# Yukayo/MobGT

Measured on AMD Instinct MI355X. Metric: check-ins/sec (train step), higher is better.
Workload: dtype bf16

## Files before the change

### __graft_entry__.py

```python
import os
import subprocess
import sys

ROOT = os.path.dirname(os.path.abspath(__file__))
if ROOT not in sys.path:
    sys.path.insert(0, ROOT)


def build() -> None:
    from mobgt_amd import _native
    for library in _native.LIBRARIES:
        library.build()
        library.lib()
    from mobgt_amd import _pairbins
    _pairbins.LIBRARY.build()
    _pairbins.LIBRARY.lib()
    from mobgt_amd import _universe
    _universe.LIBRARY.build()
    _universe.LIBRARY.lib()
    from mobgt_amd import _checkins
    _checkins.LIBRARY.build()
    _checkins.LIBRARY.lib()
    from mobgt_amd import _prefixes
    _prefixes.LIBRARY.build()
    _prefixes.LIBRARY.lib()
    from mobgt_amd import _baseline
    _baseline.LIBRARY.build()
    _baseline.LIBRARY.lib()
    from mobgt_amd import _prior
    _prior.LIBRARY.build()
    _prior.LIBRARY.lib()
    from mobgt_amd import _geoprior
    _geoprior.LIBRARY.build()
    _geoprior.LIBRARY.lib()
    from mobgt_amd import _priorfit
    _priorfit.LIBRARY.build()
    _priorfit.LIBRARY.lib()
    from mobgt_amd import _ctxprior
    _ctxprior.LIBRARY.build()
    _ctxprior.LIBRARY.lib()
    from mobgt_amd import _tokhost
    _tokhost.LIBRARY.build()
    _tokhost.LIBRARY.lib()
    from mobgt_amd import _visitprior
    _visitprior.LIBRARY.build()
    _visitprior.LIBRARY.lib()
    subprocess.check_call(["make", "-s", "-C", os.path.join(ROOT, "oracle")])
    import mobgt_amd


def smoke() -> None:
    import numpy as np
    import torch
    from mobgt_amd import ops, synth
    from mobgt_amd.model_fqandtoyo import EncoderLayer
    from oracle import algos_oracle as ao
    from oracle import model_oracle as mo
    assert torch.cuda.is_available(), "smoke() needs cuda:0"
    dev = "cuda:0"
    G, H, T, C = 3, 8, 37, 192
    torch.manual_seed(0)
    layer = EncoderLayer(C, 256, 0.1, 0.1, H).eval()
    sd = {"L." + k: v.detach().clone().requires_grad_(True) for k, v in layer.state_dict().items()}
    rng = np.random.RandomState(0)
    x = torch.from_numpy(rng.standard_normal((G, T, C)).astype(np.float32))
    gy = torch.from_numpy(rng.standard_normal((G, T, C)).astype(np.float32))
    bias = torch.from_numpy((rng.standard_normal((G, H, T, T)) * 0.5).astype(np.float32))
    bias[1, :, :, 30:] = float("-inf")
    xr, br = x.clone().requires_grad_(True), bias.clone().requires_grad_(True)
    ref = mo.encoder_layer_fq(sd, "L", xr, br, H)
    ref.backward(gy)
    layer = layer.to(dev)
    xd, bd = x.to(dev).requires_grad_(True), bias.to(dev).requires_grad_(True)
    out = layer(xd, bd)
    out.backward(gy.to(dev))
    torch.cuda.synchronize()

    def close(name, got, want, tol):
        got, want = got.detach().float().cpu().numpy(), want.detach().numpy()
# ... 40 lines not shown
```

### mobgt_amd/csrc/sgemm_body.h

```cpp
#pragma once
#include "common.h"
#include "mobgt_hip.h"

namespace mobgt_sgemm {

typedef __attribute__((ext_vector_type(4))) float f32x4;

struct SgemmParams {
    const float* A; int64_t lda;
    const float* B; int64_t ldb;
    const float* bias;
    void* C; int64_t ldc;
    int c_bf16;
    int M, N, K;
    int act;
    float slope;
    uint32_t thr;
    float inv_keep;
    uint64_t seed;
    const uint64_t* seed_dev;
    uint32_t salt;
    const float* amask;
    float mpos, mneg, mzero;
    bf16_t* ct;
// ... 45 lines not shown
        acc = __builtin_amdgcn_mfma_f32_16x16x4f32(a_r[u].w, b_r[u].w, acc, 0, 0, 0);
    }
#pragma unroll
    for (int v = 0; v < 4; ++v) part[wave][(4 * kq + v) * 17 + i] = acc[v];
    __syncthreads();
    if (wave == 0) {
    const uint64_t seed = p.thr ? p.seed + (p.seed_dev ? *p.seed_dev : 0ull) : 0ull;
    const int c = i;
    const float bv = (p.bias && c < p.N) ? p.bias[c] : 0.f;
#pragma unroll
    for (int v = 0; v < 4; ++v) {
        const int r = m0 + 4 * kq + v;
        if (r >= p.M || c >= p.N) continue;
        float o = bv;
#pragma unroll
        for (int w = 0; w < KS; ++w) o += part[w][(4 * kq + v) * 17 + i];
        if (p.act) {
            o = o > 0.f ? o : p.slope * o;
            if (p.thr) {
                const uint32_t rowh = dropout_row_hash(seed, (uint32_t)r ^ p.salt);
                o = dropout_bits16(seed, rowh, (uint32_t)c) >= p.thr ? o * p.inv_keep : 0.f;
            }
        }
        if (p.C) {
            if (p.c_bf16) reinterpret_cast<bf16_t*>(p.C)[(int64_t)r * p.ldc + c] = (bf16_t)o;
            else reinterpret_cast<float*>(p.C)[(int64_t)r * p.ldc + c] = o;
        }
        if (p.ct) p.ct[(int64_t)c * p.ldt + r] = (bf16_t)(p.ct_scale ? o * p.ct_scale[r] : o);
    }
    }
    __syncthreads();
}

}
```

### mobgt_amd/forms.py

```python
import contextlib
import os
from collections import namedtuple

Form = namedtuple("Form", "name env default doc")

_ROWS = (
    Form("safe_forms", "MOBGT_SAFE_FORMS", False, "no launch waits for peer workgroups: one workgroup per row block, the head as "
         "three launches, the GCN layer by layer (what TrainStep.guarded_step switches to before it re-runs a faulted step)"),
    Form("chain", "MOBGT_NO_CHAIN", True, "out-proj -> LN -> FFN -> LN -> the next layer's QKV in one launch (off: separate launches)"),
    Form("chain_big", "MOBGT_NO_CHAIN_BIG", True, "past 4 096 rows: the 64-row forward chain (off: the library's GEMMs)"),
    Form("chain_bwd", None, True, "the same chain backwards, d(out) -> d(attention out)"),
    Form("ln_gemm", None, True, "dropout+residual+LN as the prologue of the GEMM that consumes it (off: the two-launch form)"),
    Form("ln_gemm_bwd", "MOBGT_LN_GEMM_BWD", False, "the LayerNorm-prologue GEMMs in the backward as well"),
    Form("own_gemm", None, True, "the layer's GEMMs on csrc/gemm.hip (off: through torch)"),
    Form("tail", None, True, "a layer's input-gradient GEMM rides in its grouped weight-gradient launch"),
    Form("defer_tail", "MOBGT_NO_DEFER_TAIL", True, "a layer leaves dx and its weight gradients to the chain_bwd launch of the layer "
         "below (off: it finishes its own backward)"),
    Form("wgrad_big", None, True, "past 4 096 rows: the layer's weight gradients as one launch"),
    Form("skinny_all", "MOBGT_SKINNY_ALL", False, "all three classifier products on csrc/skinny.hip (off: dW / db only)"),
    Form("token_fwd_chain", "MOBGT_NO_TOKEN_FWD_CHAIN", True, "the encoder input's forward as one launch (off: four)"),
    Form("token_bwd_chain", "MOBGT_NO_TOKEN_BWD_CHAIN", True, "the encoder input's backward as one launch, csrc/tokbwd.hip (off: three)"),
    Form("l0_token_host", "MOBGT_NO_L0_TOKEN_HOST", True, "the first encoder layer leaves dx and its weight gradients to the encoder "
         "input's one-launch backward (off: it finishes its own backward); no workgroup waits for another, so safe_forms keeps it"),
    Form("l0_token_host_eager", "MOBGT_L0_TOKEN_HOST_EAGER", False, "l0_token_host outside a graph capture as well (off: only a step "
         "that is being captured defers; an eager step is bound by the host, gains nothing and keeps its launch list)"),
    Form("pack_passenger", "MOBGT_NO_PACK_PASSENGER", True, "the layers' weight pack, in the next front launch"),
    Form("front_passengers", "MOBGT_NO_FRONT_PASSENGERS", True, "hop table forward and node-feature indices, in the category GCN's forward"),
    Form("bias_bwd_passenger", "MOBGT_NO_BIAS_BWD_PASSENGER", True, "short batches: the bias tables' backward, in the category GCN's backward"),
    Form("bias_bwd_beside", None, True, "long batches: the bias tables' backward on a side stream (off: where autograd reaches it)"),
    Form("l0_ride", "MOBGT_NO_L0_RIDE", True, "the distance GCN's first product, in the bias assembly's launch"),
    Form("psum_defer", "MOBGT_NO_PSUM_DEFER", True, "split-K partial sums, in the step's one reduction launch into the gradient sinks"),
    Form("small_gcn", "MOBGT_NO_SMALL_GCN", True, "the three-layer category GCN as one launch each way (off: layer by layer)"),
    Form("conv_act", "MOBGT_NO_CONV_ACT", True, "bias + LeakyReLU + dropout in the small GEMM's epilogue (off: launch per product)"),
    Form("dist_gcn_fused", "MOBGT_NO_DIST_GCN_FUSED", True, "the distance GCN on the masked-GEMM launches"),
    Form("sp_gather", None, True, "sparse adjacency, transposed product as a gather (off: the atomic scatter)"),
    Form("stock_front", "MOBGT_NO_STOCK_FRONT", True, "hop table, weight pack and encoder input as one front launch"),
    Form("stock_tail", "MOBGT_NO_STOCK_TAIL", True, "the encoder input's and the wide hop table's backward share one grid at the flush"),
    Form("stock_ln_qkv", "MOBGT_NO_STOCK_LN_QKV", True, "the first layer's norm inside its QKV GEMM"),
    Form("attn_one_pass", "MOBGT_ATTN_TWO_PASS", True, "T > 64, bf16: one-pass backward (off: the two deterministic passes)"),
    Form("ddp_overlap", "MOBGT_DDP_OVERLAP", False, "the backward split into graphs, finished gradient slices all-reduced beside the next"),
    Form("ddp_host_exchange", "MOBGT_DDP_HOST_EXCHANGE", False, "all-reduce issued by the host between backward and optimizer graph"),
    Form("force_comm", "MOBGT_FORCE_COMM", False, "a process group of one rank takes the data-parallel path (tests)"),
)
_BY_NAME = {row.name: row for row in _ROWS}
_OVERRIDES = {}


def _env_set(var):
    v = os.environ.get(var, "")
    if v in ("", "0"):
        return False
    if v == "1":
        return True
    raise ValueError(f"{var}={v!r}: expected unset, '', '0' or '1'")


def on(name):
    row = _BY_NAME[name]
# ... 30 lines not shown
```

### mobgt_amd/modelGNN.py

```python
import math

import torch
import torch.nn as nn
import torch.nn.functional as F
from torch.nn import Parameter

from . import forms
from .step_state import STEP


def mm_tn_splitk(x, g, max_chunks=32, bf16_operands=False, dw=None):
    if (bf16_operands and x.is_cuda and x.dtype == torch.float32 and g.dtype == torch.float32 and x.shape[1] % 2 == 0
            and g.shape[1] % 2 == 0 and x.is_contiguous() and g.is_contiguous()
            and x.data_ptr() % 8 == 0 and g.data_ptr() % 8 == 0):
        from . import ops
        return ops.linear_wgrad(x, g, leaf=True, dw=dw)[0]
    P = x.shape[0]
    s = max((c for c in range(1, max_chunks + 1) if P % c == 0), default=1)
    if s == 1 or P < 2048:
        return x.t() @ g
    return torch.bmm(x.view(s, P // s, -1).transpose(1, 2), g.view(s, P // s, -1)).sum(0)


_OUT_DTYPE = [None]
# ... 447 lines not shown
                  _p(t2), *[_p(x) for x in grads], _p(scratch[n * H1:]), _p(scratch[:n * H1]),
                  _p(counter), n, K0, H1, H2, H3, slope, p_drop, seed, _p(seed_dev), salt,
                  *extra, _stream())
        if job is not None:
            job["done"] = outs
        return (None, None, None, *grads, None, None, None, None, None, None)


class _DistGcnFn(torch.autograd.Function):

    @staticmethod
    def forward(ctx, ax_pad, mask, mask_t, scale, rows, w0, b0, w1, b1, w2, b2, slope, p_drop, seed, seed_dev, salt):
        from . import ops, _lib
        from .ops import _p, _stream
        P, R, NO = ax_pad.shape[0], rows.numel(), w2.shape[1]
        dev = ax_pad.device
        y0t = xt_workspace(dev, P, 16, slot=0)
        y0 = ops.small_gemm(ax_pad, w0, b0, leaky=slope, k_b=w0.shape[0], ct=(y0t, None, False))
        y1t = xt_workspace(dev, P, 64, slot=0)
        t1 = torch.empty(P, 16, dtype=torch.float32, device=dev)
        y1 = torch.empty(P, 64, dtype=torch.float32, device=dev)
        u = torch.empty(R, 64, dtype=torch.float32, device=dev)
        parts = torch.empty(4, R, NO, dtype=torch.float32, device=dev)
        rs_rows = torch.empty(R, dtype=torch.float32, device=dev)
        _lib.call("mobgt_mask_gemm_l1_fwd", _p(mask), mask.shape[1], _p(scale), _p(y0t), y0t.stride(0), _p(t1), _p(w1), _p(b1),
                  float(slope), float(p_drop), int(seed), _p(seed_dev), int(salt) & 0xFFFFFFFF, _p(y1),
                  _p(y1t), y1t.stride(0), None, 0, P, P, _stream())
        _lib.call("mobgt_mask_rows_fwd", _p(mask), mask.shape[1], _p(rows), _p(scale), _p(y1t), y1t.stride(0), _p(w2), _p(b2),
                  _p(u), _p(parts), _p(rs_rows), R, P, NO, _stream())
        ctx.save_for_backward(ax_pad, y0, t1, y1, u, rs_rows, rows, w0, w1, w2, mask_t, scale)
        ctx.mv0, ctx.mv1 = ops.act_mask_values(slope, 0.0), ops.act_mask_values(slope, p_drop)
        ctx.sinks = tuple(ops.grad_sink(t) for t in (w0, b0, w1, b1, w2, b2))
        p0, rest = parts[0], parts[1:]
        ctx.mark_non_differentiable(rest)
        ctx.set_materialize_grads(False)
        return p0, rest

    @staticmethod
    def backward(ctx, g, _g_rest=None):
        from . import ops, _lib
        from .ops import _p, _stream
        ax_pad, y0, t1, y1, u, rs_rows, rows, w0, w1, w2, mask_t, scale = ctx.saved_tensors
        k_w0, k_b0, k_w1, k_b1, k_w2, k_b2 = ctx.sinks
        if g is None:
            return (None,) * 16
        g = g.contiguous()
        dev = g.device
        P, R = ax_pad.shape[0], rows.numel()

        def dst(k, n):
            return k[:] if k is not None else ops.zeros_f32((n,), dev)
        db2 = dst(k_b2, w2.shape[1])
        dW2 = ops.linear_wgrad_masked(u, g, db=db2, db_of_x=True, leaf=True, dw=k_w2[:] if k_w2 is not None else None)
        gut = xt_workspace(dev, R, 64, slot=2)
        ops.small_gemm(g, w2, b_is_nk=True, ct=(gut, rs_rows, True))
        dy1 = torch.empty(P, 64, dtype=torch.float32, device=dev)
        dtt = xt_workspace(dev, P, 16, slot=1)
        _lib.call("mobgt_mask_rows_bwd", _p(mask_t), mask_t.shape[1], _p(rows), _p(gut), gut.stride(0), _p(y1),
                  float(ctx.mv1[0]), float(ctx.mv1[1]), float(ctx.mv1[2]), _p(w1), _p(scale), _p(dy1),
                  _p(dtt), dtt.stride(0), R, P, _stream())
        db1 = dst(k_b1, 64)
        dW1 = ops.linear_wgrad_masked(t1, dy1, x_mask=y1, mask_vals=ctx.mv1, db=db1, db_of_x=True, leaf=True,
                                      dw=k_w1[:] if k_w1 is not None else None)
        dy0 = mask_gemm(MaskAdj(None, mask_t, scale), None, transposed=True, xt=dtt)
        db0 = dst(k_b0, 16)
        dw_dst = None
        extra = (ax_pad.shape[1] - w0.shape[0]) * w0.shape[1]
        if k_w0 is not None and k_w0.is_contiguous() and 0 <= extra <= 16:
            dw_dst = torch.as_strided(k_w0, (ax_pad.shape[1], w0.shape[1]), (w0.shape[1], 1))
        dW0 = ops.linear_wgrad_masked(ax_pad, dy0, x_mask=y0, mask_vals=ctx.mv0, db=db0, db_of_x=True, leaf=True, dw=dw_dst)
        dW0 = dW0[:w0.shape[0]]
        return (None, None, None, None, None, dW0, db0[:], dW1, db1[:], dW2, db2[:], None, None, None, None, None)


def _dist_gcn_ok(gcn, adj_x_pad, rows, mask_adj):
    if not forms.on("dist_gcn_fused") or adj_x_pad is None or rows is None or mask_adj is None or len(gcn.gcn) != 3:
        return False
    g0, g1, g2 = gcn.gcn
    if not (adj_x_pad.is_cuda and adj_x_pad.dtype == torch.float32 and adj_x_pad.is_contiguous() and adj_x_pad.shape[1] % 16 == 0
            and 0 <= adj_x_pad.shape[1] - g0.in_features < 16):
        return False
    if (g0.out_features, g1.in_features, g1.out_features, g2.in_features) != (16, 16, 64, 64) or g2.out_features % 4 or g2.out_features > 192:
        return False
    for g in (g0, g1, g2):
        if g.bias is None or g.weight.dtype != torch.float32 or not g.weight.is_contiguous() or not g.bias.is_contiguous():
            return False
    P = adj_x_pad.shape[0]
    if rows.dtype != torch.int64 or not rows.is_contiguous() or rows.numel() < 1 or mask_adj.scale.numel() != P:
# ... 16 lines not shown
        n_hidden = len(self.gcn) - 1
        adj_x_pad = None
        if adj_x is not None and adj_x.shape[1] != self.gcn[0].in_features:
            adj_x_pad, adj_x = adj_x, adj_x[:, :self.gcn[0].in_features]
        if rows is None and mask_adj is None and x.is_cuda and _small_gcn_ok(self, x, adj, adj_x, adj_t):
            from . import ops
            p_drop = self.dropout if self.training else 0.0
            g0, g1, g2 = self.gcn
            salt = (0x2000 + g2.out_features) & 0xFFFFFFFF
            pre = STEP.gcn_prelaunched.pop(id(self), None)
            seed_dev = ops.dropout_seed(0.0)[1]
            if pre is not None and (pre[0][0], pre[0][2], pre[0][3]) == (float(p_drop), id(seed_dev), salt):
                seed = pre[0][1]
            else:
                seed, seed_dev = ops.dropout_seed(p_drop)
                if pre is not None:
                    if pre[1][2] is not None:
                        torch.cuda.current_stream().wait_event(pre[1][2])
                    pre = None
            with torch.autocast(device_type="cuda", enabled=False):
                return _SmallGcnFn.apply(adj_x, adj, adj_t, g0.weight, g0.bias, g1.weight, g1.bias, g2.weight, g2.bias,
                                         float(self.leaky_relu.negative_slope), float(p_drop), seed, seed_dev, salt,
                                         pre[1] if pre is not None else None)
        ax_in = adj_x_pad if adj_x_pad is not None else adj_x
        if x.is_cuda and not isinstance(adj, CsrAdj) and _dist_gcn_ok(self, ax_in, rows, mask_adj):
            from . import ops
            p_drop = self.dropout if self.training else 0.0
            seed, seed_dev = ops.dropout_seed(p_drop)
            g0, g1, g2 = self.gcn
            with torch.autocast(device_type="cuda", enabled=False):
                p0, rest = _DistGcnFn.apply(ax_in, mask_adj.mask, mask_adj.mask_t, mask_adj.scale, rows, g0.weight, g0.bias,
                                            g1.weight, g1.bias, g2.weight, g2.bias, float(self.leaky_relu.negative_slope),
                                            float(p_drop), seed, seed_dev, 0x2000 + g2.out_features)
            if parts_ok:
                p0._mobgt_parts = tuple(rest.unbind(0))
                return p0
            return ((p0 + rest[0]) + rest[1]) + rest[2]
        if x.is_cuda and all(g.out_features % 4 == 0 and g.bias is not None for g in self.gcn[:-1]):
            from . import ops
            for i in range(n_hidden):
                p_drop = self.dropout if (i == n_hidden - 1 and self.training) else 0.0
                salt = 0x2000 + self.gcn[-1].out_features
                gc = self.gcn[i]
                pre = adj_x if i == 0 else None
                pre_pad = adj_x_pad if i == 0 else None
                if (pre_pad is not None and mask_adj is not None and not isinstance(adj, CsrAdj) and i + 1 < n_hidden
                        and pre_pad.dtype == torch.float32 and pre_pad.is_contiguous() and pre_pad.shape[1] % 16 == 0
                        and 0 <= pre_pad.shape[1] - gc.in_features < 16 and gc.bias is not None and gc.out_features in (16, 32, 48, 64)
                        and gc.weight.is_contiguous() and forms.on("conv_act")
                        and _conv_act_ok(gc.out_features, self.gcn[i + 1].weight, self.gcn[i + 1].bias)):
                    seed, seed_dev = ops.dropout_seed(p_drop)
                    yt = xt_workspace(pre_pad.device, pre_pad.shape[0], gc.out_features, slot=0)
                    with torch.autocast(device_type="cuda", enabled=False):
                        x = _ConvActFn.apply(None, pre_pad, gc.weight, gc.bias, None, float(self.leaky_relu.negative_slope),
                                             float(p_drop), seed, seed_dev, salt, ops.OutRef(yt))
                    x._mobgt_xt = yt
                    continue
                if (pre is None and mask_adj is not None and not isinstance(adj, CsrAdj) and x.dtype == torch.float32
                        and _mask_conv_ok(x, gc.weight) and _conv_act_ok(x.shape[1], gc.weight, gc.bias)):
                    seed, seed_dev = ops.dropout_seed(p_drop)
                    xt = getattr(x, "_mobgt_xt", None)
                    with torch.autocast(device_type="cuda", enabled=False):
                        x = _ConvActFn.apply(None if pre is not None else x, pre, gc.weight, gc.bias, mask_adj,
                                             float(self.leaky_relu.negative_slope), float(p_drop), seed, seed_dev, salt,
                                             ops.OutRef(xt) if xt is not None else None)
                    continue
# ... 29 lines not shown
```

### mobgt_amd/model_fqandtoyo.py

```python
import os
import pickle

import numpy as np
import torch
import torch.nn as nn
import torch.nn.functional as F

from . import forms, ops
from .restriction import Restriction
from .step_state import STEP
from .lr import PolynomialDecayLR
from .model import (FeedForwardNetwork, MultiHeadAttention, hop_table_from, no_grad_row0, fused_layer_forward,
                    refresh_shadows, flush_pending_pack)
from .modelGNN import GCN, prelaunch_small_gcn

node_dim = 2000


def freedman_diaconis_bins(x, return_bins=False):
    iqr = np.subtract(*np.percentile(x, [75, 25]))
    binsize = 2 * iqr * np.power(len(x), -1 / 3)
    bins = np.ceil((np.max(x) - np.min(x)) / binsize)
    if return_bins:
        return int(bins), np.histogram(x, int(bins))[1]
# ... 276 lines not shown
            hop = self.hop_table(batched_data)
        return ops.build_bias(batched_data.attn_bias, batched_data.rel_pos, batched_data.poi_pos, edge_input,
                              self.rel_pos_encoder.weight, self.poi_pos_encoder.weight, hop,
                              self.graph_token_virtual_distance.weight, D, dtype=self.bias_dtype)

    def node_features(self, batched_data, indices=None):
        G, N = batched_data.x.shape[:2]
        idx, real, rows_only = indices if indices is not None else self.gather_indices(batched_data)
        poi_idx, time_idx, cat_idx, pos_idx, gcn_rows, zero_idx, in_deg, out_deg = idx.unbind(0)
        if self.sparse_adj:
            from .modelGNN import CsrAdj
            adj = CsrAdj(self.D_A_rowptr, self.D_A_col, self.D_A_val, self.D_AT_rowptr, self.D_AT_col, self.D_AT_val)
            poidist = self.poi_distance_model(self.X, adj, self.D_AX, rows=gcn_rows.reshape(-1) if rows_only else None)
        else:
            mask_adj = None
            if getattr(self, "D_mask", None) is not None:
                from .modelGNN import MaskAdj
                mask_adj = MaskAdj(self.D_mask, self.D_mask_t, self.D_scale)
            poidist = self.poi_distance_model(self.X, self.D_A, self.D_AX, rows=gcn_rows.reshape(-1) if rows_only else None,
                                              adj_t=self.D_A_T, mask_adj=mask_adj, parts_ok=G * N <= 4096)
        ops.trace_nan("poidist", poidist)
        catemb = self.poi_cat_model(self.C_X, self.C_A, self.C_AX, adj_t=self.C_A_T)
        Wp, Wt, Wc, C = poidist.shape[1], self.time_embed_model_48.weight.shape[1], catemb.shape[1], self.pos_embed.pe.shape[1]
        f4 = self.embed_fuse_model4
        one_launch = G * N <= 4096
        l0 = self.layers[0]
        first_qkv = None
        if (getattr(l0, "fused", False) and getattr(l0, "_packed_fresh", False) and getattr(l0, "act_dtype", None) == torch.bfloat16
                and not torch.is_autocast_enabled("cuda")):
            first_qkv = (l0._packed[0], l0._shadows[1])
        ops.token_fwd_deferral(one_launch and first_qkv is not None and self.act_dtype == torch.bfloat16 and C == 192 and Wp + Wt == 160)
        try:
            return self._node_features_tail(batched_data, G, N, poidist, catemb, real, one_launch, first_qkv, Wp, Wt, Wc, C,
                                            poi_idx, time_idx, cat_idx, pos_idx, zero_idx, in_deg, out_deg)
        finally:
            ops.token_fwd_deferral(False)

    def _node_features_tail(self, batched_data, G, N, poidist, catemb, real, one_launch, first_qkv, Wp, Wt, Wc, C,
                            poi_idx, time_idx, cat_idx, pos_idx, zero_idx, in_deg, out_deg):
        f4 = self.embed_fuse_model4
        if one_launch:
            pt, x4, add = ops.embed_gather_multi(
                [(poidist, poi_idx, 0, 0, False, None)] +
                [(part, poi_idx, 0, 0, 2, None) for part in getattr(poidist, "_mobgt_parts", ())] +
                [(self.time_embed_model_48.weight, time_idx, 0, Wp, False, self.time_embed_model_48.padding_idx),
                 (catemb, cat_idx, 1, Wp + Wt, False, None),
                 (self.fre_embed_model.weight, zero_idx, 2, 0, False, 0), (self.in_degree_encoder.weight, in_deg, 2, 0, True, 0),
                 (self.out_degree_encoder.weight, out_deg, 2, 0, True, 0), (self.pos_embed.pe, pos_idx, 2, 0, True, None)],
                [Wp + Wt, Wp + Wt + Wc, C])
            f2 = ops.linear_splitk(pt, self.embed_fuse_model2.fuse_embed.weight, self.embed_fuse_model2.fuse_embed.bias,
                                   self.act_dtype == torch.bfloat16, slope=self.embed_fuse_model2.leaky_relu.negative_slope,
                                   out=x4[:, :Wp + Wt])
            if f2.data_ptr() == x4.data_ptr():
                x4 = ops.join_cols(x4, f2)
            else:
                x4 = torch.cat((f2, x4[:, Wp + Wt:]), 1)
            nf = ops.linear_splitk(x4, f4.fuse_embed.weight, f4.fuse_embed.bias, getattr(f4, "bf16_wgrad", False),
                                   slope=f4.leaky_relu.negative_slope)
            if f2.data_ptr() == x4.data_ptr() and self.act_dtype == torch.bfloat16 and getattr(f4, "bf16_wgrad", False):
                ops.register_token_chain(nf, x4, Wp + Wt, f4.fuse_embed.weight, f4.leaky_relu.negative_slope,
                                         self.embed_fuse_model2.fuse_embed.weight, self.embed_fuse_model2.leaky_relu.negative_slope)
        else:
            pt = ops.embed_gather_concat([poidist, self.time_embed_model_48.weight], [poi_idx, time_idx],
                                         padding_idx=[None, self.time_embed_model_48.padding_idx])
            f2 = ops.linear_splitk(pt, self.embed_fuse_model2.fuse_embed.weight, self.embed_fuse_model2.fuse_embed.bias,
                                   self.act_dtype == torch.bfloat16, slope=self.embed_fuse_model2.leaky_relu.negative_slope)
            nf = f4(f2, ops.embed_gather_sum([catemb], [cat_idx]))
            add = ops.embed_gather_sum(
                [self.fre_embed_model.weight, self.in_degree_encoder.weight, self.out_degree_encoder.weight, self.pos_embed.pe],
                [zero_idx, in_deg, out_deg, pos_idx], padding_idx=[0, 0, 0, None])
        ops.trace_nan("pt", pt)
        ops.trace_nan("f2", f2)
        ops.trace_nan("fuse4", nf)
        return ops.assemble_tokens(nf.view(G, N, -1), real, add.view(G, N, -1), self.graph_token.weight, self.pos_embed.pe, self.pos_embed.dropout.p,
                                   self.input_dropout.p, self.training,
                                   bf16_copy=self.act_dtype == torch.bfloat16 and getattr(self.layers[0], "fused", False),
                                   pe_row0_via_gather=one_launch, first_qkv=first_qkv)

    def validate_batch(self, batched_data):
        if getattr(batched_data, "_mobgt_validated", None) is self or not batched_data.x.is_cuda:
            return
        if torch.cuda.is_current_stream_capturing():
# ... 187 lines not shown
```

### mobgt_amd/ops.py

```python
import contextlib
import ctypes
import math

import torch

from . import _lib, _tokhost, forms
from ._lib import F32, BF16, I64, I32, I16, U8, check
from .step_state import STEP

_DT = {torch.float32: F32, torch.bfloat16: BF16}
BIAS_LONG_PAIRS, HOP_DMAX, TOPK_MAX = _lib.LIBRARY.constants("BIAS_LONG_PAIRS", "HOP_DMAX", "TOPK_MAX_K")
SKINNY_MAX_G, SKINNY_MAX_K, SKINNY_MFMA_MAX_K, SKINNY_MFMA_K_STEP = _lib.LIBRARY.constants(
    "SKINNY_MAX_G", "SKINNY_MAX_K", "SKINNY_MFMA_MAX_K", "SKINNY_MFMA_K_STEP")
_IT = {torch.int64: I64, torch.int32: I32, torch.int16: I16, torch.uint8: U8}


def _stream():
    return ctypes.c_void_p(torch.cuda.current_stream().cuda_stream)


def _p(t):
    return ctypes.c_void_p(t.data_ptr()) if t is not None else ctypes.c_void_p(0)


def _require_cuda(*ts):
    for t in ts:
        if t is not None and not t.is_cuda:
            raise RuntimeError("mobgt_amd ops run on the GPU only (there is no CPU fallback); got a CPU tensor")




def _ws_word(ws, off):
    return ws.view(torch.int32)[off // 4:off // 4 + 1]


def _scrub_exchange_area(ws, fault_off):
    ws[fault_off + 4:].zero_()
    torch.cuda.synchronize()
# ... 1151 lines not shown
                  _IT[ctx.idx[0].dtype], _stream())
        return (None, None, *grads, *([None] * n))


def embed_gather_concat(tables, indices, padding_idx=None):
    _require_cuda(*tables, *indices)
    n = len(tables)
    shape = indices[0].shape
    skip = tuple(-1 if (padding_idx is None or padding_idx[t] is None) else int(padding_idx[t]) for t in range(n))
    idx = [i.contiguous().reshape(-1) for i in indices]
    tabs = [t.float().contiguous() for t in tables]
    out = _GatherConcatFn.apply(skip, n, *tabs, *idx)
    return out.view(*shape, out.shape[1])


_ROW0_PENDING = {}


def token_fwd_deferral(on):
    flush_token_fwd()
    STEP.token_fwd_on = bool(on) and forms.on("token_fwd_chain") and not _NAN_TRACE["on"]


def flush_token_fwd():
    for k in ("gather", "f2", "f4"):
        rec = STEP.token_fwd.pop(k, None)
        if rec is not None:
            rec["launch"]()


class _GatherMultiFn(torch.autograd.Function):

    @staticmethod
    def forward(ctx, spec, out_widths, n, *args):
        tables, idx = args[:n], args[n:]
        R = idx[0].numel()
        dev = tables[0].device
        outs = [torch.empty(R, w, dtype=torch.float32, device=dev) for w in out_widths]
        ci, i64, vp = ctypes.c_int, ctypes.c_int64, ctypes.c_void_p

        def launch():
            _lib.call("mobgt_embed_gather_multi",
                n, _ptr_array(tables), None, _ptr_array(idx), (i64 * n)(*[sp[3] for sp in spec]),
                (ci * n)(*[t.shape[1] for t in tables]), (ci * n)(*[sp[1] for sp in spec]), (ci * n)(*[int(sp[2]) for sp in spec]),
                (vp * n)(*[outs[sp[0]].data_ptr() for sp in spec]), (i64 * n)(*[outs[sp[0]].stride(0) for sp in spec]), R,
                _IT[idx[0].dtype], 0, None, 0, _stream())
        if STEP.token_fwd_on and "gather" not in STEP.token_fwd and len(outs) == 3 and all(i_.dtype == idx[0].dtype for i_ in idx):
            STEP.token_fwd["gather"] = dict(launch=launch, tables=tables, idx=idx, spec=spec, outs=outs, R=R)
        else:
            launch()
        ctx.idx, ctx.spec, ctx.n = idx, spec, n
        ctx.ptrs = [t.data_ptr() for t in tables]
        ctx.shapes = [t.shape for t in tables]
        ctx.sinks = [grad_sink(t) for t in tables]
        return tuple(outs)

    @staticmethod
    def backward(ctx, *douts):
        n, spec = ctx.n, ctx.spec
        dev = ctx.idx[0].device
        R = ctx.idx[0].numel()
        gbuf = []
        for g in douts:
            if g is not None and (g.stride(1) != 1 or g.stride(0) % 4 or g.data_ptr() % 16 or g.dtype != torch.float32):
                g = g.float().contiguous()
            gbuf.append(g)
        grads = [(ctx.sinks[t][:] if ctx.sinks[t] is not None else zeros_f32(tuple(sh), dev))
                 if (ctx.needs_input_grad[3 + t] and gbuf[spec[t][0]] is not None) else None for t, sh in enumerate(ctx.shapes)]
        jobs = [t for t in range(n) if grads[t] is not None]
        if jobs:
            m = len(jobs)
            ci, i64, vp = ctypes.c_int, ctypes.c_int64, ctypes.c_void_p
            extra, extra_job = None, 0
            for k, t in enumerate(jobs):
                pend = _ROW0_PENDING.pop(ctx.ptrs[t], None)
                if pend is not None:
                    extra, extra_job = pend, k
            _lib.call("mobgt_embed_gather_multi",
                m, None, (vp * m)(*[grads[t].data_ptr() for t in jobs]), (vp * m)(*[ctx.idx[t].data_ptr() for t in jobs]),
                (i64 * m)(*[spec[t][3] for t in jobs]), (ci * m)(*[ctx.shapes[t][1] for t in jobs]),
                (ci * m)(*[spec[t][1] for t in jobs]), None, (vp * m)(*[gbuf[spec[t][0]].data_ptr() for t in jobs]),
                (i64 * m)(*[gbuf[spec[t][0]].stride(0) for t in jobs]), R, _IT[ctx.idx[0].dtype], 1, _p(extra), extra_job,
                _stream())
        return (None, None, None, *grads, *([None] * n))


def embed_gather_multi(jobs, out_widths):
    n = len(jobs)
    tabs = [j[0].float().contiguous() for j in jobs]
    idx = [j[1].contiguous().reshape(-1) for j in jobs]
    _require_cuda(*tabs, *idx)
    spec = tuple((int(j[2]), int(j[3]), int(j[4]), -1 if j[5] is None else int(j[5])) for j in jobs)
    for k, sp in enumerate(spec):
        assert sp[2] != 2 or (k > 0 and tabs[k].shape[1] == tabs[k - 1].shape[1] and not tabs[k].requires_grad
                              and (k < 4 or any(s_[2] != 2 for s_ in spec[k - 3:k]))), "fold job (at most three per gather)"
    return list(_GatherMultiFn.apply(spec, tuple(out_widths), n, *tabs, *idx))


class _JoinColsFn(torch.autograd.Function):

    @staticmethod
    def forward(ctx, whole, part):
        ctx.w = part.shape[1]
        return whole.detach().view_as(whole)

    @staticmethod
    def backward(ctx, g):
        return g, g[:, :ctx.w]


def join_cols(whole, part):
    return _JoinColsFn.apply(whole, part)


class _GradientTailLossFn(torch.autograd.Function):
    @staticmethod
    def forward(ctx, logits, targets, alpha, target_offset):
        logits = logits.float().contiguous()
        G, V = logits.shape
        dlogits = torch.empty_like(logits)
        loss = torch.empty((), dtype=torch.float32, device=logits.device)
        _lib.call("mobgt_gradient_tail_loss", _p(logits), _p(targets.long().contiguous()), int(target_offset), _p(dlogits),
                  _p(loss), G, V, float(alpha), _stream())
        ctx.save_for_backward(dlogits)
        return loss

    @staticmethod
    def backward(ctx, g):
        (dlogits,) = ctx.saved_tensors
# ... 976 lines not shown
```

### mobgt_amd/step_state.py

```python
import contextlib
from collections import namedtuple

PARKED, CARRIED, SWITCH = "parked", "carried", "switch"
Field = namedtuple("Field", "name scope new doc")
_none = type(None)

FIELDS = (
    Field("zero_arena", SWITCH, _none, "TrainStep._prologue sets the step's ZeroArena; ops.zeros_f32 carves from it"),
    Field("grad_sinks", CARRIED, dict, "TrainStep (ops.set_grad_sinks): parameter address -> (weak parameter, gradient view); ops.grad_sink reads"),
    Field("sink_census", SWITCH, lambda: {"on": False, "cur": {}, "max": {}}, "train.used_parameters' dry run counts ops.grad_sink requests per forward"),
    Field("bias_bwd_job", PARKED, _none, "_BuildBiasFn.forward parks; the category GCN's backward launch, the side stream or its own backward takes"),
    Field("front_on", SWITCH, bool, "the model's forward (ops.front_deferral) around the hop table and the node indices"),
    Field("front_hop", PARKED, _none, "_HopTableFn.forward parks; the category GCN's / stock front's forward launch or ops.flush_front takes"),
    Field("front_ni", PARKED, _none, "ops.node_index parks; the same launches take"),
    Field("token_fwd_on", SWITCH, bool, "model_fqandtoyo.node_features (ops.token_fwd_deferral)"),
    Field("token_fwd", PARKED, dict, "'gather' / 'f2' / 'f4': _GatherMultiFn / _LinearSplitKFn.forward record; _AssembleTokensFn launches them as one"),
    Field("token_fwd_fused_calls", CARRIED, int, "how often mobgt_token_fwd_chain took the three records (a counter for tests)"),
    Field("token_chain", CARRIED, _none, "ops.register_token_chain: the encoder-input chain of the forward that just ran; its backward reads it"),
    Field("token_pending", PARKED, dict, "_AssembleTokensFn.backward parks under a gradient's address (with the first layer's tail, taken from layer_tails, "
          "under 'tail'); FuseEmbeddings-4 / -2's backward re-park / launch"),
    Field("front_sgemm", PARKED, dict, "'job': ops.front_small_gemm parks, the bias assembly's launch takes; 'done': its result until ops.small_gemm asks"),
    Field("wgrad_on", SWITCH, bool, "ops.recording_wgrads around the trainer's backward"),
    Field("wgrad_items", PARKED, list, "leaf weight gradients (ops.linear_wgrad*, fused layers) for ops.flush_deferred_wgrads' grouped launch"),
    Field("wgrad_hop", PARKED, _none, "_HopTableFn.backward parks; rides in the flush's first grouped launch"),
    Field("wgrad_hop_wide", PARKED, _none, "_HopTableFn.backward past 256 edge ids; shares the flush's stock tail launch"),
    Field("wgrad_stock_tok", PARKED, _none, "_StockTokensFn.backward parks; the flush's stock tail launch takes"),
    Field("wgrad_psum", PARKED, list, "ops.defer_partial_sum: split-K partial sums for the flush's one reduction launch"),
    Field("layer_tails", PARKED, dict, "(graph task, device, address of dx1) -> a fused layer's tail; the chain launch of the layer below (first layer: "
          "the encoder input's backward) takes"),
    Field("tail_check_task", PARKED, _none, "graph task whose end-of-backward check (fused_layer._pending_check) is queued"),
    Field("weight_pack", PARKED, list, "model.pack_layer_weights(defer=True) parks; the category GCN's / stock front's forward launch takes"),
    Field("gcn_prelaunched", PARKED, dict, "modelGNN.prelaunch_small_gcn: id(module) -> (key, result); that module's forward adopts it"),
)


class StepState:
    def __init__(self):
        for f in FIELDS:
            setattr(self, f.name, f.new())

    def leftovers(self):
        held = {f.name: getattr(self, f.name) for f in FIELDS if f.scope == PARKED}
        return {k: sorted(map(str, v)) if isinstance(v, dict) else len(v) if isinstance(v, list) else type(v).__name__
                for k, v in held.items() if v is not None and v != [] and v != {}}
# ... 25 lines not shown
```

Baseline: 27230.

## Fuse token-gradient scatters into one burst kernel with distance GCN gu product riding along

Result: faster. 27710 (median of 6 runs) (+1.7%).

```diff
diff --git a/__graft_entry__.py b/__graft_entry__.py
--- a/__graft_entry__.py
+++ b/__graft_entry__.py
@@ -45,6 +45,9 @@
     from mobgt_amd import _visitprior
     _visitprior.LIBRARY.build()
     _visitprior.LIBRARY.lib()
+    from mobgt_amd import _tokscatter
+    _tokscatter.LIBRARY.build()
+    _tokscatter.LIBRARY.lib()
     subprocess.check_call(["make", "-s", "-C", os.path.join(ROOT, "oracle")])
     import mobgt_amd
 
diff --git a/include/mobgt_tokscatter.h b/include/mobgt_tokscatter.h
--- /dev/null
+++ b/include/mobgt_tokscatter.h
@@ -0,0 +1,31 @@
+#ifndef MOBGT_TOKSCATTER_H
+#define MOBGT_TOKSCATTER_H
+#include <stdint.h>
+
+#ifdef __cplusplus
+extern "C" {
+#endif
+
+#define MOBGT_TOKSCATTER_EBADDIM (-1)
+#define MOBGT_TOKSCATTER_EALIGN (-2)
+#define MOBGT_TOKSCATTER_EDTYPE (-3)
+
+#define MOBGT_TOKSCATTER_ABI_VERSION 1
+int mobgt_tokscatter_abi_version(void);
+
+#define MOBGT_TOKSCATTER_I64 0
+#define MOBGT_TOKSCATTER_I32 1
+#define MOBGT_TOKSCATTER_MAX_JOBS 8
+#define MOBGT_TOKSCATTER_MAX_WIDTH 192
+#define MOBGT_TOKSCATTER_RIDE_MAX_K 192
+#define MOBGT_TOKSCATTER_RIDE_MAX_N 64
+
+int mobgt_tokscatter_bwd(int n, float* const* d_tables, const void* const* idx, const int64_t* skip, const int* width,
+                         const int* coff, const float* const* buf, const int64_t* ld, int64_t R, int idx_dtype,
+                         const float* extra_row0, int extra_job, int identity_job, const float* ride_w, int64_t ride_ldw,
+                         const float* ride_scale, void* ride_gut, int64_t ride_ldt, int ride_n, void* stream);
+
+#ifdef __cplusplus
+}
+#endif
+#endif
diff --git a/mobgt_amd/_tokscatter.py b/mobgt_amd/_tokscatter.py
--- /dev/null
+++ b/mobgt_amd/_tokscatter.py
@@ -0,0 +1,16 @@
+from ._native import Library, NativeError
+
+
+class MobgtTokscatterError(NativeError):
+    pass
+
+
+LIBRARY = Library("mobgt_tokscatter.h", "csrc_tokscatter", "libmobgt_tokscatter.so", "MOBGT_TOKSCATTER_", error=MobgtTokscatterError,
+                  missing="the burst scatter runs on the device only (MOBGT_NO_SCATTER_BURST=1 does without).",
+                  errors={"EBADDIM": "size outside the supported limits, null buffer, or an identity job / ride that cannot be",
+                          "EALIGN": "pointer or stride violates the documented alignment", "EDTYPE": "unknown index dtype code"},
+                  extra_inputs=("csrc/sgemm_body.h", "csrc/common.h"))
+lib, launch = LIBRARY.lib, LIBRARY.launch
+SIGNATURES, CONSTANTS, ABI_VERSION = LIBRARY.SIGNATURES, LIBRARY.CONSTANTS, LIBRARY.ABI_VERSION
+MAX_JOBS, MAX_WIDTH, RIDE_MAX_K, RIDE_MAX_N = LIBRARY.constants("MAX_JOBS", "MAX_WIDTH", "RIDE_MAX_K", "RIDE_MAX_N")
+EBADDIM, EALIGN, EDTYPE = LIBRARY.constants("EBADDIM", "EALIGN", "EDTYPE")
diff --git a/mobgt_amd/csrc/sgemm_body.h b/mobgt_amd/csrc/sgemm_body.h
--- a/mobgt_amd/csrc/sgemm_body.h
+++ b/mobgt_amd/csrc/sgemm_body.h
@@ -101,4 +101,49 @@
     __syncthreads();
 }
 
+constexpr int NK_MAXS = 12;
+template <typename TI>
+__device__ __forceinline__ void sgemm_nk_tile_burst(const SgemmParams& p, const int tile, const TI* row_idx, const int64_t skip) {
+    const int lane = threadIdx.x & 63;
+    const int i = lane & 15, kq = lane >> 4;
+    const int tiles_n = (p.N + 15) / 16;
+    const int m0 = (tile / tiles_n) * 16, n0 = (tile % tiles_n) * 16;
+    const int ra = min(m0 + i, p.M - 1);
+    const float* arow = p.A + (int64_t)ra * p.lda + 4 * kq;
+    const float* brow = p.B + (int64_t)min(n0 + i, p.N - 1) * p.ldb + 4 * kq;
+    const int nsteps = p.K / 16;
+    const TI ri_raw = row_idx ? row_idx[ra] : (TI)0;
+    float4 a_r[NK_MAXS], b_r[NK_MAXS];
+#pragma unroll
+    for (int s = 0; s < NK_MAXS; ++s) {
+        const int sc = min(s, nsteps - 1);
+        a_r[s] = *reinterpret_cast<const float4*>(arow + 16 * sc);
+        b_r[s] = *reinterpret_cast<const float4*>(brow + 16 * sc);
+    }
+    float sc_r[4];
+#pragma unroll
+    for (int v = 0; v < 4; ++v) sc_r[v] = p.ct_scale ? p.ct_scale[min(m0 + 4 * kq + v, p.M - 1)] : 1.f;
+    const int64_t ri = (int64_t)ri_raw;
+    const uint32_t keep = (ri < 0 || ri == skip) ? 0u : 0xFFFFFFFFu;
+    f32x4 acc = f32x4{0.f, 0.f, 0.f, 0.f};
+#pragma unroll
+    for (int s = 0; s < NK_MAXS; ++s) {
+        if (s < nsteps) {
+            acc = __builtin_amdgcn_mfma_f32_16x16x4f32(__uint_as_float(__float_as_uint(a_r[s].x) & keep), b_r[s].x, acc, 0, 0, 0);
+            acc = __builtin_amdgcn_mfma_f32_16x16x4f32(__uint_as_float(__float_as_uint(a_r[s].y) & keep), b_r[s].y, acc, 0, 0, 0);
+            acc = __builtin_amdgcn_mfma_f32_16x16x4f32(__uint_as_float(__float_as_uint(a_r[s].z) & keep), b_r[s].z, acc, 0, 0, 0);
+            acc = __builtin_amdgcn_mfma_f32_16x16x4f32(__uint_as_float(__float_as_uint(a_r[s].w) & keep), b_r[s].w, acc, 0, 0, 0);
+        }
+    }
+    const int c = n0 + i;
+#pragma unroll
+    for (int v = 0; v < 4; ++v) {
+        const int r = m0 + 4 * kq + v;
+        if (r < p.M && c < p.N) {
+            const float o = acc[v] + 0.f;
+            p.ct[(int64_t)c * p.ldt + r] = (bf16_t)(p.ct_scale ? o * sc_r[v] : o);
+        }
+    }
 }
+
+}
diff --git a/mobgt_amd/csrc_tokscatter/tokscatter.hip b/mobgt_amd/csrc_tokscatter/tokscatter.hip
--- /dev/null
+++ b/mobgt_amd/csrc_tokscatter/tokscatter.hip
@@ -0,0 +1,140 @@
+#include "mobgt_tokscatter.h"
+#include "sgemm_body.h"
+
+namespace {
+
+constexpr int MAXJ = MOBGT_TOKSCATTER_MAX_JOBS;
+constexpr int NPIECE = MOBGT_TOKSCATTER_MAX_WIDTH / 64;
+static_assert(MOBGT_TOKSCATTER_MAX_WIDTH % 64 == 0, "whole pieces");
+static_assert(MOBGT_TOKSCATTER_RIDE_MAX_K == 16 * mobgt_sgemm::NK_MAXS, "the k-steps the ride's tile holds in flight");
+static_assert(MOBGT_TOKSCATTER_EBADDIM == MOBGT_EBADDIM && MOBGT_TOKSCATTER_EALIGN == MOBGT_EALIGN &&
+              MOBGT_TOKSCATTER_EDTYPE == MOBGT_EDTYPE && MOBGT_TOKSCATTER_I64 == MOBGT_I64 && MOBGT_TOKSCATTER_I32 == MOBGT_I32,
+              "the codes of include/mobgt_hip.h");
+
+struct ScatterParams {
+    float* d_tables[MAXJ];
+    const void* idx[MAXJ];
+    int64_t skip[MAXJ];
+    int width[MAXJ];
+    const float* src[MAXJ];
+    int64_t ld[MAXJ];
+    int64_t R;
+    const float* extra_src;
+    float* extra_dst;
+    int extra_width, identity;
+    const void* ride_idx;
+    int64_t ride_skip;
+    int row_blocks;
+    int ride_tiles;
+    mobgt_sgemm::SgemmParams ride;
+};
+
+template <typename TI>
+__global__ __launch_bounds__(256) void scatter_burst_kernel(const ScatterParams p) {
+    const int lane = threadIdx.x & 63, wave = __builtin_amdgcn_readfirstlane(threadIdx.x >> 6);
+    if ((int)blockIdx.x >= p.row_blocks) {
+        const int tile = ((int)blockIdx.x - p.row_blocks) * 4 + wave;
+        if (tile < p.ride_tiles)
+            mobgt_sgemm::sgemm_nk_tile_burst(p.ride, tile, reinterpret_cast<const TI*>(p.ride_idx), p.ride_skip);
+        return;
+    }
+    const int64_t r = (int64_t)blockIdx.x * 4 + wave;
+    if (r >= p.R) return;
+    int64_t row[MAXJ];
+#pragma unroll
+    for (int t = 0; t < MAXJ; ++t) row[t] = (int64_t)reinterpret_cast<const TI*>(p.idx[t])[r];
+    float v[MAXJ][NPIECE], ex[NPIECE];
+#pragma unroll
+    for (int t = 0; t < MAXJ; ++t) {
+        const float* from = p.src[t] + r * p.ld[t];
+#pragma unroll
+        for (int k = 0; k < NPIECE; ++k) v[t][k] = from[max(min(lane + 64 * k, p.width[t] - 1), 0)];
+    }
+#pragma unroll
+    for (int k = 0; k < NPIECE; ++k) ex[k] = p.extra_src[min(lane + 64 * k, p.extra_width - 1)];
+    float* dt[MAXJ];
+    int64_t sk[MAXJ];
+    int wd[MAXJ];
+#pragma unroll
+    for (int t = 0; t < MAXJ; ++t) {
+        dt[t] = p.d_tables[t]; sk[t] = p.skip[t]; wd[t] = p.width[t];
+        asm volatile("" : "+s"(dt[t]), "+s"(sk[t]), "+s"(wd[t]));
+    }
+#if defined(__HIP_DEVICE_COMPILE__) && !defined(__gfx950__) && !defined(__gfx942__) && !defined(__gfx90a__)
+#error "scatter_burst_kernel: the s_waitcnt immediate below is the gfx9 encoding"
+#endif
+    __builtin_amdgcn_s_waitcnt(0x0F70);
+    if (p.extra_dst && blockIdx.x == 0 && wave == 0) {
+#pragma unroll
+        for (int k = 0; k < NPIECE; ++k)
+            if (lane + 64 * k < p.extra_width) atomicAdd(p.extra_dst + lane + 64 * k, ex[k]);
+    }
+#pragma unroll
+    for (int t = 0; t < MAXJ; ++t) {
+        if (!dt[t]) continue;
+        const bool live = row[t] >= 0 && row[t] != sk[t];
+        if (t == p.identity) {
+            float* dst = dt[t] + r * wd[t];
+#pragma unroll
+            for (int k = 0; k < NPIECE; ++k)
+                if (lane + 64 * k < wd[t]) dst[lane + 64 * k] = live ? v[t][k] : 0.f;
+        } else if (live) {
+            float* dst = dt[t] + row[t] * wd[t];
+#pragma unroll
+            for (int k = 0; k < NPIECE; ++k)
+                if (lane + 64 * k < wd[t]) atomicAdd(dst + lane + 64 * k, v[t][k]);
+        }
+    }
+}
+
+}
+
+extern "C" int mobgt_tokscatter_abi_version(void) { return MOBGT_TOKSCATTER_ABI_VERSION; }
+
+extern "C" int mobgt_tokscatter_bwd(int n, float* const* d_tables, const void* const* idx, const int64_t* skip, const int* width,
+                                    const int* coff, const float* const* buf, const int64_t* ld, int64_t R, int idx_dtype,
+                                    const float* extra_row0, int extra_job, int identity_job, const float* ride_w, int64_t ride_ldw,
+                                    const float* ride_scale, void* ride_gut, int64_t ride_ldt, int ride_n, void* stream) {
+    if (n < 1 || n > MAXJ || !d_tables || !idx || !width || !coff || !buf || !ld) return MOBGT_TOKSCATTER_EBADDIM;
+    if (idx_dtype != MOBGT_TOKSCATTER_I64 && idx_dtype != MOBGT_TOKSCATTER_I32) return MOBGT_TOKSCATTER_EDTYPE;
+    if (identity_job < -1 || identity_job >= n || (identity_job >= 0 && !d_tables[identity_job])) return MOBGT_TOKSCATTER_EBADDIM;
+    if (extra_row0 && (extra_job < 0 || extra_job >= n || extra_job == identity_job)) return MOBGT_TOKSCATTER_EBADDIM;
+    if (R > (int64_t)1 << 30) return MOBGT_TOKSCATTER_EBADDIM;
+    ScatterParams p = {};
+    for (int t = 0; t < n; ++t) {
+        if (width[t] < 1 || width[t] > MOBGT_TOKSCATTER_MAX_WIDTH || coff[t] < 0 || ld[t] < (int64_t)coff[t] + width[t] || !buf[t] || !idx[t])
+            return MOBGT_TOKSCATTER_EBADDIM;
+        if (((uintptr_t)buf[t] | (uintptr_t)d_tables[t]) & 3) return MOBGT_TOKSCATTER_EALIGN;
+        p.d_tables[t] = d_tables[t]; p.idx[t] = idx[t]; p.skip[t] = skip ? skip[t] : -1;
+        p.width[t] = width[t]; p.src[t] = buf[t] + coff[t]; p.ld[t] = ld[t];
+    }
+    for (int t = n; t < MAXJ; ++t) {
+        p.idx[t] = p.idx[n - 1]; p.src[t] = p.src[n - 1]; p.ld[t] = p.ld[n - 1]; p.skip[t] = -1;
+    }
+    p.R = R; p.identity = identity_job;
+    p.extra_src = p.src[0]; p.extra_width = 1;
+    if (extra_row0) {
+        if ((uintptr_t)extra_row0 & 3) return MOBGT_TOKSCATTER_EALIGN;
+        p.extra_src = extra_row0; p.extra_width = width[extra_job]; p.extra_dst = d_tables[extra_job];
+    }
+    p.row_blocks = (int)((R + 3) / 4);
+    if (ride_gut) {
+        const int j = identity_job;
+        if (j < 0 || !ride_w || ride_n < 1 || ride_n > MOBGT_TOKSCATTER_RIDE_MAX_N || (width[j] & 15) ||
+            width[j] > MOBGT_TOKSCATTER_RIDE_MAX_K || ride_ldw < width[j] || ride_ldt < R)
+            return MOBGT_TOKSCATTER_EBADDIM;
+        if ((((uintptr_t)p.src[j] | (uintptr_t)ride_w) & 15) || (ld[j] & 3) || (ride_ldw & 3) || ((uintptr_t)ride_gut & 1) ||
+            ((uintptr_t)ride_scale & 3))
+            return MOBGT_TOKSCATTER_EALIGN;
+        mobgt_sgemm::SgemmParams& s = p.ride;
+        s.A = p.src[j]; s.lda = ld[j]; s.B = ride_w; s.ldb = ride_ldw; s.M = (int)R; s.N = ride_n; s.K = width[j]; s.Kb = s.K;
+        s.ct = reinterpret_cast<bf16_t*>(ride_gut); s.ldt = ride_ldt; s.ct_scale = ride_scale;
+        p.ride_tiles = (int)((R + 15) / 16) * ((ride_n + 15) / 16);
+        p.ride_idx = idx[j]; p.ride_skip = p.skip[j];
+    }
+    if (R <= 0) return 0;
+    const dim3 grid((unsigned)(p.row_blocks + (p.ride_tiles + 3) / 4)), block(256);
+    if (idx_dtype == MOBGT_TOKSCATTER_I64) hipLaunchKernelGGL(scatter_burst_kernel<int64_t>, grid, block, 0, (hipStream_t)stream, p);
+    else hipLaunchKernelGGL(scatter_burst_kernel<int32_t>, grid, block, 0, (hipStream_t)stream, p);
+    return (int)hipGetLastError();
+}
diff --git a/mobgt_amd/forms.py b/mobgt_amd/forms.py
--- a/mobgt_amd/forms.py
+++ b/mobgt_amd/forms.py
@@ -24,6 +24,14 @@
          "input's one-launch backward (off: it finishes its own backward); no workgroup waits for another, so safe_forms keeps it"),
     Form("l0_token_host_eager", "MOBGT_L0_TOKEN_HOST_EAGER", False, "l0_token_host outside a graph capture as well (off: only a step "
          "that is being captured defers; an eager step is bound by the host, gains nothing and keeps its launch list)"),
+    Form("scatter_burst", "MOBGT_NO_SCATTER_BURST", True, "short batches, fused distance GCN: the encoder input's gradients are scattered "
+         "in one burst per position, the distance GCN's compact table written instead of scattered (off: job after job); no workgroup "
+         "waits for another, so safe_forms keeps it"),
+    Form("scatter_burst_eager", "MOBGT_SCATTER_BURST_EAGER", False, "scatter_burst outside a graph capture as well (off: only a step "
+         "that is being captured takes it; an eager step keeps its launch list)"),
+    Form("dist_gu_ride", "MOBGT_NO_DIST_GU_RIDE", True, "the distance GCN's backward product gu, in the burst scatter's launch (needs "
+         "scatter_burst); no workgroup waits for another, so safe_forms keeps it"),
+    Form("dist_gu_ride_eager", "MOBGT_DIST_GU_RIDE_EAGER", False, "dist_gu_ride outside a graph capture as well (with scatter_burst_eager)"),
     Form("pack_passenger", "MOBGT_NO_PACK_PASSENGER", True, "the layers' weight pack, in the next front launch"),
     Form("front_passengers", "MOBGT_NO_FRONT_PASSENGERS", True, "hop table forward and node-feature indices, in the category GCN's forward"),
     Form("bias_bwd_passenger", "MOBGT_NO_BIAS_BWD_PASSENGER", True, "short batches: the bias tables' backward, in the category GCN's backward"),
diff --git a/mobgt_amd/modelGNN.py b/mobgt_amd/modelGNN.py
--- a/mobgt_amd/modelGNN.py
+++ b/mobgt_amd/modelGNN.py
@@ -503,6 +503,7 @@
         ctx.mv0, ctx.mv1 = ops.act_mask_values(slope, 0.0), ops.act_mask_values(slope, p_drop)
         ctx.sinks = tuple(ops.grad_sink(t) for t in (w0, b0, w1, b1, w2, b2))
         p0, rest = parts[0], parts[1:]
+        ctx.gu_job = ops.park_dist_gu_job(p0, w2, rs_rows, xt_workspace(dev, R, 64, slot=2), R, NO) if any(ctx.needs_input_grad) else None
         ctx.mark_non_differentiable(rest)
         ctx.set_materialize_grads(False)
         return p0, rest
@@ -513,6 +514,7 @@
         from .ops import _p, _stream
         ax_pad, y0, t1, y1, u, rs_rows, rows, w0, w1, w2, mask_t, scale = ctx.saved_tensors
         k_w0, k_b0, k_w1, k_b1, k_w2, k_b2 = ctx.sinks
+        rode = ops.take_dist_gu_job(ctx.gu_job)
         if g is None:
             return (None,) * 16
         g = g.contiguous()
@@ -524,7 +526,8 @@
         db2 = dst(k_b2, w2.shape[1])
         dW2 = ops.linear_wgrad_masked(u, g, db=db2, db_of_x=True, leaf=True, dw=k_w2[:] if k_w2 is not None else None)
         gut = xt_workspace(dev, R, 64, slot=2)
-        ops.small_gemm(g, w2, b_is_nk=True, ct=(gut, rs_rows, True))
+        if not rode:
+            ops.small_gemm(g, w2, b_is_nk=True, ct=(gut, rs_rows, True))
         dy1 = torch.empty(P, 64, dtype=torch.float32, device=dev)
         dtt = xt_workspace(dev, P, 16, slot=1)
         _lib.call("mobgt_mask_rows_bwd", _p(mask_t), mask_t.shape[1], _p(rows), _p(gut), gut.stride(0), _p(y1),
@@ -607,6 +610,8 @@
                 p0, rest = _DistGcnFn.apply(ax_in, mask_adj.mask, mask_adj.mask_t, mask_adj.scale, rows, g0.weight, g0.bias,
                                             g1.weight, g1.bias, g2.weight, g2.bias, float(self.leaky_relu.negative_slope),
                                             float(p_drop), seed, seed_dev, 0x2000 + g2.out_features)
+            if not p0.requires_grad:
+                STEP.dist_gu_job = None
             if parts_ok:
                 p0._mobgt_parts = tuple(rest.unbind(0))
                 return p0
diff --git a/mobgt_amd/model_fqandtoyo.py b/mobgt_amd/model_fqandtoyo.py
--- a/mobgt_amd/model_fqandtoyo.py
+++ b/mobgt_amd/model_fqandtoyo.py
@@ -332,12 +332,12 @@
         ops.token_fwd_deferral(one_launch and first_qkv is not None and self.act_dtype == torch.bfloat16 and C == 192 and Wp + Wt == 160)
         try:
             return self._node_features_tail(batched_data, G, N, poidist, catemb, real, one_launch, first_qkv, Wp, Wt, Wc, C,
-                                            poi_idx, time_idx, cat_idx, pos_idx, zero_idx, in_deg, out_deg)
+                                            poi_idx, time_idx, cat_idx, pos_idx, zero_idx, in_deg, out_deg, rows_only)
         finally:
             ops.token_fwd_deferral(False)
 
     def _node_features_tail(self, batched_data, G, N, poidist, catemb, real, one_launch, first_qkv, Wp, Wt, Wc, C,
-                            poi_idx, time_idx, cat_idx, pos_idx, zero_idx, in_deg, out_deg):
+                            poi_idx, time_idx, cat_idx, pos_idx, zero_idx, in_deg, out_deg, rows_only=False):
         f4 = self.embed_fuse_model4
         if one_launch:
             pt, x4, add = ops.embed_gather_multi(
@@ -347,7 +347,8 @@
                  (catemb, cat_idx, 1, Wp + Wt, False, None),
                  (self.fre_embed_model.weight, zero_idx, 2, 0, False, 0), (self.in_degree_encoder.weight, in_deg, 2, 0, True, 0),
                  (self.out_degree_encoder.weight, out_deg, 2, 0, True, 0), (self.pos_embed.pe, pos_idx, 2, 0, True, None)],
-                [Wp + Wt, Wp + Wt + Wc, C])
+                [Wp + Wt, Wp + Wt + Wc, C],
+                identity=0 if (rows_only and hasattr(poidist, "_mobgt_parts") and poidist.shape[0] == G * N) else None)
             f2 = ops.linear_splitk(pt, self.embed_fuse_model2.fuse_embed.weight, self.embed_fuse_model2.fuse_embed.bias,
                                    self.act_dtype == torch.bfloat16, slope=self.embed_fuse_model2.leaky_relu.negative_slope,
                                    out=x4[:, :Wp + Wt])
diff --git a/mobgt_amd/ops.py b/mobgt_amd/ops.py
--- a/mobgt_amd/ops.py
+++ b/mobgt_amd/ops.py
@@ -4,7 +4,7 @@
 
 import torch
 
-from . import _lib, _tokhost, forms
+from . import _lib, _tokhost, _tokscatter, forms
 from ._lib import F32, BF16, I64, I32, I16, U8, check
 from .step_state import STEP
 
@@ -1222,7 +1222,7 @@
 class _GatherMultiFn(torch.autograd.Function):
 
     @staticmethod
-    def forward(ctx, spec, out_widths, n, *args):
+    def forward(ctx, spec, out_widths, n, identity, *args):
         tables, idx = args[:n], args[n:]
         R = idx[0].numel()
         dev = tables[0].device
@@ -1240,6 +1240,9 @@
         else:
             launch()
         ctx.idx, ctx.spec, ctx.n = idx, spec, n
+        ctx.identity = identity if (identity is not None and tables[identity].shape[0] == R and not spec[identity][2]) else None
+        ctx.burst = (ctx.identity is not None and forms.on("scatter_burst")
+                     and (torch.cuda.is_current_stream_capturing() or forms.on("scatter_burst_eager")))
         ctx.ptrs = [t.data_ptr() for t in tables]
         ctx.shapes = [t.shape for t in tables]
         ctx.sinks = [grad_sink(t) for t in tables]
@@ -1255,10 +1258,17 @@
             if g is not None and (g.stride(1) != 1 or g.stride(0) % 4 or g.data_ptr() % 16 or g.dtype != torch.float32):
                 g = g.float().contiguous()
             gbuf.append(g)
-        grads = [(ctx.sinks[t][:] if ctx.sinks[t] is not None else zeros_f32(tuple(sh), dev))
-                 if (ctx.needs_input_grad[3 + t] and gbuf[spec[t][0]] is not None) else None for t, sh in enumerate(ctx.shapes)]
-        jobs = [t for t in range(n) if grads[t] is not None]
-        if jobs:
+        wanted = [bool(ctx.needs_input_grad[4 + t] and gbuf[spec[t][0]] is not None) for t in range(n)]
+        jobs = [t for t in range(n) if wanted[t]]
+        burst = (ctx.burst and 1 <= len(jobs) <= _tokscatter.MAX_JOBS and ctx.idx[0].dtype in (torch.int64, torch.int32)
+                 and all(ctx.idx[t].dtype == ctx.idx[0].dtype and ctx.shapes[t][1] <= _tokscatter.MAX_WIDTH for t in jobs))
+        ident = ctx.identity if (burst and ctx.identity in jobs and ctx.sinks[ctx.identity] is None) else None
+        grads = [(ctx.sinks[t][:] if ctx.sinks[t] is not None else
+                  torch.empty(tuple(sh), dtype=torch.float32, device=dev) if t == ident else zeros_f32(tuple(sh), dev))
+                 if wanted[t] else None for t, sh in enumerate(ctx.shapes)]
+        if jobs and burst:
+            _scatter_burst(ctx, jobs, grads, gbuf, ident, R)
+        elif jobs:
             m = len(jobs)
             ci, i64, vp = ctypes.c_int, ctypes.c_int64, ctypes.c_void_p
             extra, extra_job = None, 0
@@ -1272,10 +1282,50 @@
                 (ci * m)(*[spec[t][1] for t in jobs]), None, (vp * m)(*[gbuf[spec[t][0]].data_ptr() for t in jobs]),
                 (i64 * m)(*[gbuf[spec[t][0]].stride(0) for t in jobs]), R, _IT[ctx.idx[0].dtype], 1, _p(extra), extra_job,
                 _stream())
-        return (None, None, None, *grads, *([None] * n))
-
-
-def embed_gather_multi(jobs, out_widths):
+        return (None, None, None, None, *grads, *([None] * n))
+
+
+def _scatter_burst(ctx, jobs, grads, gbuf, ident, R):
+    spec, m = ctx.spec, len(jobs)
+    ci, i64, vp = ctypes.c_int, ctypes.c_int64, ctypes.c_void_p
+    extra, extra_job = None, 0
+    for k, t in enumerate(jobs):
+        pend = _ROW0_PENDING.pop(ctx.ptrs[t], None)
+        if pend is not None:
+            extra, extra_job = pend, k
+    ride = (None, 0, None, None, 0, 0)
+    job = STEP.dist_gu_job
+    if job is not None and ident is not None:
+        g, coff, no = gbuf[spec[ident][0]], spec[ident][1], ctx.shapes[ident][1]
+        if (job["out_ptr"] == ctx.ptrs[ident] and job["R"] == R and job["NO"] == no and no % 16 == 0 and no <= _tokscatter.RIDE_MAX_K
+                and job["w2"].shape[0] <= _tokscatter.RIDE_MAX_N and (g.data_ptr() + 4 * coff) % 16 == 0 and g.stride(0) % 4 == 0
+                and job["w2"].is_contiguous() and job["w2"].data_ptr() % 16 == 0 and job["gut"].stride(0) >= R):
+            STEP.dist_gu_job = None
+            job["taken"] = True
+            ride = (_p(job["w2"]), job["w2"].stride(0), _p(job["rs_rows"]), _p(job["gut"]), job["gut"].stride(0), job["w2"].shape[0])
+    _tokscatter.launch("mobgt_tokscatter_bwd",
+        m, (vp * m)(*[grads[t].data_ptr() for t in jobs]), (vp * m)(*[ctx.idx[t].data_ptr() for t in jobs]),
+        (i64 * m)(*[spec[t][3] for t in jobs]), (ci * m)(*[ctx.shapes[t][1] for t in jobs]), (ci * m)(*[spec[t][1] for t in jobs]),
+        (vp * m)(*[gbuf[spec[t][0]].data_ptr() for t in jobs]), (i64 * m)(*[gbuf[spec[t][0]].stride(0) for t in jobs]), R,
+        _IT[ctx.idx[0].dtype], _p(extra), extra_job, jobs.index(ident) if ident is not None else -1, *ride, _stream())
+
+
+def take_dist_gu_job(job):
+    if STEP.dist_gu_job is job:
+        STEP.dist_gu_job = None
+    return bool(job is not None and job.get("taken"))
+
+
+def park_dist_gu_job(out, w2, rs_rows, gut, R, NO):
+    STEP.dist_gu_job = None
+    if not (forms.on("dist_gu_ride") and forms.on("scatter_burst")
+            and (torch.cuda.is_current_stream_capturing() or (forms.on("dist_gu_ride_eager") and forms.on("scatter_burst_eager")))):
+        return None
+    STEP.dist_gu_job = job = dict(out_ptr=out.data_ptr(), w2=w2.detach(), rs_rows=rs_rows, gut=gut, R=int(R), NO=int(NO))
+    return job
+
+
+def embed_gather_multi(jobs, out_widths, identity=None):
     n = len(jobs)
     tabs = [j[0].float().contiguous() for j in jobs]
     idx = [j[1].contiguous().reshape(-1) for j in jobs]
@@ -1284,7 +1334,7 @@
     for k, sp in enumerate(spec):
         assert sp[2] != 2 or (k > 0 and tabs[k].shape[1] == tabs[k - 1].shape[1] and not tabs[k].requires_grad
                               and (k < 4 or any(s_[2] != 2 for s_ in spec[k - 3:k]))), "fold job (at most three per gather)"
-    return list(_GatherMultiFn.apply(spec, tuple(out_widths), n, *tabs, *idx))
+    return list(_GatherMultiFn.apply(spec, tuple(out_widths), n, identity, *tabs, *idx))
 
 
 class _JoinColsFn(torch.autograd.Function):
diff --git a/mobgt_amd/step_state.py b/mobgt_amd/step_state.py
--- a/mobgt_amd/step_state.py
+++ b/mobgt_amd/step_state.py
@@ -10,6 +10,7 @@
     Field("grad_sinks", CARRIED, dict, "TrainStep (ops.set_grad_sinks): parameter address -> (weak parameter, gradient view); ops.grad_sink reads"),
     Field("sink_census", SWITCH, lambda: {"on": False, "cur": {}, "max": {}}, "train.used_parameters' dry run counts ops.grad_sink requests per forward"),
     Field("bias_bwd_job", PARKED, _none, "_BuildBiasFn.forward parks; the category GCN's backward launch, the side stream or its own backward takes"),
+    Field("dist_gu_job", PARKED, _none, "_DistGcnFn.forward parks (ops.park_dist_gu_job); the encoder input's burst scatter takes, or that node's own backward drops"),
     Field("front_on", SWITCH, bool, "the model's forward (ops.front_deferral) around the hop table and the node indices"),
     Field("front_hop", PARKED, _none, "_HopTableFn.forward parks; the category GCN's / stock front's forward launch or ops.flush_front takes"),
     Field("front_ni", PARKED, _none, "ops.node_index parks; the same launches take"),
```
